# ConwayBeyond/Funscript-Flow

Measured on AMD Instinct MI355X. Metric: 1080p frame-pairs/sec, higher is better.
Workload: dtype f32

## Files before the change

### funscript_flow_amd/csrc/ffl_api.hip

```cpp
#include "../../include/ffl.h"
#include "ffl_kernels.h"

#include <math.h>
#include <stdarg.h>
#include <stdio.h>
#include <string.h>

#include <algorithm>
#include <condition_variable>
#include <mutex>
#include <string>
#include <thread>
#include <vector>

#define FFL_EV_RING 16
#define FFL_RAW_RING 4

template <class H, class Arg, hipError_t (*Free)(Arg)>
struct Owned {
    H h = H();
    Owned() = default;
    explicit Owned(H take) : h(take) {}
    Owned(Owned &&o) noexcept : h(o.release()) {}
    Owned &operator=(Owned &&o) noexcept { std::swap(h, o.h); return *this; }
// ... 671 lines not shown
            HIPCHK(c, hipMemcpyAsync(rb.d, rb.h, fbytes, hipMemcpyHostToDevice, c->s_copy));
        }
        {
            ProfScope ps(c, FFL_K_FRONTEND, c->s_copy);
            if (rp) ffl_launch_frontend_remap(desc(rb.d), c->d_gray + (size_t)fs * c->N, fp, *rp, c->s_copy);
            else ffl_launch_frontend(desc(rb.d), c->d_gray + (size_t)fs * c->N, fp, c->s_copy);
        }
        HIPCHK(c, hipEventRecord(rb.ev, c->s_copy));
        rb.busy = true;
    }
    return publish_frames(c, first, n);
}

extern "C" {

int ffl_device_count(void) {
    int n = 0;
    if (hipGetDeviceCount(&n) != hipSuccess) return 0;
    return n;
}

const char *ffl_last_error(const ffl_ctx *ctx) {
    if (!ctx) return g_create_error.c_str();
    static thread_local std::string copy;
    CtxLock lk(ctx->mu);
    copy = ctx->err;
    return copy.c_str();
}

const char *ffl_kernel_name(int k) {
    static const char *names[FFL_K_COUNT] = {"k_gray",  "k_pyr_level", "k_polyexp", "k_frontend",
                                             "k_update_matrices", "k_blur_solve", "k_pass1", "k_radial"};
    return (k >= 0 && k < FFL_K_COUNT) ? names[k] : "?";
}

void ffl_destroy(ffl_ctx *c) {
    if (!c) return;
    hipSetDevice(c->device);
    for (auto &L : c->lanes)
        if (L.st) hipStreamSynchronize(L.st);
    if (c->s_post) hipStreamSynchronize(c->s_post);
    if (c->s_copy) hipStreamSynchronize(c->s_copy);
    prof_collect(c);
    c->pool.shutdown();
    delete c;
}

static int create_resources(ffl_ctx *c) {
    const int width = c->w, height = c->h, n_frame_slots = c->n_fslots, n_flow_slots = c->n_slots;
    const int num_lanes = c->opt.lanes;
    const Geometry &geo = c->geo;
    const Layout &lay = c->lay;
    HIPCHK(nullptr, hipSetDevice(c->device));
    int prio_least = 0, prio_greatest = 0;
    HIPCHK(nullptr, hipDeviceGetStreamPriorityRange(&prio_least, &prio_greatest));
    HIPCHK(nullptr, hipStreamCreateWithPriority(c->s_copy.put(), hipStreamNonBlocking, prio_greatest));
    HIPCHK(nullptr, hipStreamCreateWithPriority(c->s_post.put(), hipStreamNonBlocking, prio_greatest));
    HIPCHK_ALLOC(nullptr, hipMalloc, c->d_gray, lay.gray + 16);
    HIPCHK_ALLOC(nullptr, hipMalloc, c->d_bgr, lay.bgr);
    HIPCHK_ALLOC(nullptr, hipHostMalloc, c->h_stage_gray, lay.gray, hipHostMallocDefault);
    HIPCHK_ALLOC(nullptr, hipHostMalloc, c->h_stage_bgr, lay.bgr, hipHostMallocDefault);
    c->p1_blocks = ffl_pass1_blocks(width, height);
    c->lanes.resize(num_lanes);
    for (auto &L : c->lanes) {
        HIPCHK(nullptr, hipStreamCreateWithFlags(L.st.put(), hipStreamNonBlocking));
        HIPCHK(nullptr, L.ring.create(FFL_EV_RING));
        HIPCHK_ALLOC(nullptr, hipMalloc, L.d_I, lay.I);
        HIPCHK_ALLOC(nullptr, hipMalloc, L.d_T, lay.T);
        HIPCHK_ALLOC(nullptr, hipMalloc, L.d_R, lay.R);
        for (auto &M : L.d_M) HIPCHK_ALLOC(nullptr, hipMalloc, M, lay.M);
        HIPCHK_ALLOC(nullptr, hipMalloc, L.d_flowA, lay.flow);
        HIPCHK_ALLOC(nullptr, hipMalloc, L.d_flowB, lay.flow);
        HIPCHK_ALLOC(nullptr, hipMalloc, L.d_pkey, lay.p1);
        HIPCHK_ALLOC(nullptr, hipMalloc, L.d_psum, lay.p1);
        HIPCHK_ALLOC(nullptr, hipMalloc, L.d_tab, 1);
        HIPCHK_ALLOC(nullptr, hipHostMalloc, L.h_tab, lay.tab, hipHostMallocDefault);
        for (int k = geo.levels; k >= 0; k--, L.n_jobs++) {
            const LevelGeom &g = geo.lv[k];
            const size_t plane = (size_t)g.lw * g.lh;
            PyrJob &P = L.pyr[L.n_jobs];
            P.w = width; P.h = height; P.lw = g.lw; P.lh = g.lh;
            P.sx = (double)width / g.lw; P.sy = (double)height / g.lh;
            P.gk = g.gk;
            P.tmp = L.d_T + lay.t_off[k]; P.tmp_stride = ffl_pyr_tmp_floats(width, height, g.lw);
            P.I = L.d_I + lay.i_off[k]; P.I_stride = plane;
            PolyJob &Q = L.poly[L.n_jobs];
            Q.I = P.I; Q.I_stride = plane;
            Q.R = L.d_R + lay.r_off[k]; Q.R_stride = 5 * plane; Q.plane = plane;
            Q.w = g.lw; Q.h = g.lh;
        }
    }
    HIPCHK_ALLOC(nullptr, hipMalloc, c->d_flow, lay.slots);
    HIPCHK_ALLOC(nullptr, hipHostMalloc, c->h_res, lay.res, hipHostMallocMapped);
    HIPCHK(nullptr, hipHostGetDevicePointer((void **)&c->d_res, c->h_res, 0));
    HIPCHK_ALLOC(nullptr, hipMalloc, c->d_rpsum, (size_t)c->p1_blocks * FFL_MAXB);
    {
        std::vector<double> wy(2 * (size_t)height);
        for (int y = 0; y < height; y++) {
            wy[y] = (double)(height - y) / (double)height;
            wy[height + y] = (double)y / (double)height;
        }
        HIPCHK_ALLOC(nullptr, hipMalloc, c->d_wytab, wy.size());
        HIPCHK(nullptr, hipMemcpy(c->d_wytab, wy.data(), sizeof(double) * wy.size(), hipMemcpyHostToDevice));
    }
    HIPCHK_ALLOC(nullptr, hipMalloc, c->d_wtab, FFL_MAXB);
    HIPCHK_ALLOC(nullptr, hipHostMalloc, c->h_wtab, FFL_MAXB, hipHostMallocDefault);
// ... 2175 lines not shown
        ProfScope ps(c, FFL_K_PASS1, st);
        ffl_launch_pass1(c->d_ptab, 1, c->w, c->h, pov_mode, c->d_pskey, c->d_rpsum, st);
    }
    EvRef done;
    if (int rc = publish_post(c, 1, &slot, &done)) return rc;
    HIPCHK(c, hipGetLastError());
    return FFL_OK;
}

int ffl_submit_pair(ffl_ctx *c, int slot, const uint8_t *prev, const uint8_t *next, int width, int height, int channels,
                    ptrdiff_t stride_bytes, int pov_mode) {
    if (!c) return FFL_ERR_INVALID;
    if (!flow_slot_ok(c, slot) || 2 * slot + 1 >= c->n_fslots) {
        CtxLock lk(c->mu);
        return set_err(c, FFL_ERR_INVALID, "ffl_submit_pair: slot %d needs frame slots %d,%d and a flow slot", slot, 2 * slot, 2 * slot + 1);
    }
    int rc = ffl_upload_frame(c, 2 * slot, prev, width, height, channels, stride_bytes);
    if (rc) return rc;
    rc = ffl_upload_frame(c, 2 * slot + 1, next, width, height, channels, stride_bytes);
    if (rc) return rc;
    int f0 = 2 * slot, f1 = 2 * slot + 1;
    return ffl_flow_pairs(c, 1, &f0, &f1, &slot, pov_mode);
}

int ffl_sync(ffl_ctx *c) {
    if (!c) return FFL_ERR_INVALID;
    std::unique_lock<std::mutex> ul(c->up_mu);
    std::unique_lock<std::mutex> pl(c->post_mu);
    CtxLock lk(c->mu);
    std::vector<hipEvent_t> evs;
    evs.push_back(ev_latest(c->up_ring).get());
    for (auto &rb : c->raw)
        if (rb.busy) evs.push_back(rb.ev);
    for (auto &L : c->lanes) evs.push_back(ev_latest(L.ring).get());
    evs.push_back(ev_latest(c->post_ring).get());
    pl.unlock();
    ul.unlock();
    return wait_unlocked(c, lk, evs.data(), (int)evs.size());
}

static constexpr struct { const char *name; int value; } kFixedKnobs[] = {
    {"blur_tile_h", 16}, {"run_ahead", 0}, {"merge_expand", 1}};
static const int *fixed_knob(const char *name) {
    for (const auto &k : kFixedKnobs)
        if (!strcmp(name, k.name)) return &k.value;
    return nullptr;
}
static const FflOptionRow *option_row(const char *name) {
    for (const FflOptionRow &r : kFflOptionRows)
        if (!strcmp(name, r.name)) return &r;
    return nullptr;
}

static int set_option_impl(FflOptions &o, const char *name, int value, bool live) {
    if (const int *fixed = fixed_knob(name)) return value == *fixed ? FFL_OK : FFL_ERR_INVALID;
    const FflOptionRow *r = option_row(name);
    if (!r || value < r->lo || value > r->hi) return FFL_ERR_INVALID;
    if (live && r->member == &FflOptions::lanes) return value == o.lanes ? FFL_OK : FFL_ERR_STATE;
    o.*r->member = r->flag ? value != 0 : value;
    return FFL_OK;
}

static int get_option_impl(const FflOptions &o, const char *name, int *value) {
    const int *fixed = fixed_knob(name);
    const FflOptionRow *r = option_row(name);
    if (!fixed && !r) return FFL_ERR_INVALID;
    *value = fixed ? *fixed : o.*r->member;
    return FFL_OK;
}

int ffl_set_option(const char *name, int value) {
    if (!name) return FFL_ERR_INVALID;
    std::lock_guard<std::mutex> g(g_opt_mu);
    return set_option_impl(g_opts, name, value, false);
}

int ffl_ctx_set_option(ffl_ctx *c, const char *name, int value) {
    if (!c || !name) return FFL_ERR_INVALID;
    CtxLock lk(c->mu);
    const int rc = set_option_impl(c->opt, name, value, true);
    if (rc == FFL_OK) c->opt_epoch++;
    else if (rc == FFL_ERR_STATE) set_err(c, rc, "ffl_ctx_set_option: \"lanes\" is fixed once the context exists (%d)", c->opt.lanes);
    else set_err(c, rc, "ffl_ctx_set_option: unknown option or value out of range: %s = %d", name, value);
    return rc;
}

int ffl_ctx_get_option(ffl_ctx *c, const char *name, int *value) {
    if (!name || !value) return FFL_ERR_INVALID;
    if (!c) {
        std::lock_guard<std::mutex> g(g_opt_mu);
        return get_option_impl(g_opts, name, value);
    }
    CtxLock lk(c->mu);
    return get_option_impl(c->opt, name, value);
}

int ffl_graph_stats(ffl_ctx *c, int *captured, int *replayed, int *capture_failures) {
    if (!c) return FFL_ERR_INVALID;
    CtxLock lk(c->mu);
    if (captured) *captured = c->graph_captured;
    if (replayed) *replayed = c->graph_replayed;
    if (capture_failures) *capture_failures = c->graph_failed;
    return FFL_OK;
}

int ffl_profile_enable(ffl_ctx *c, unsigned class_mask) {
    if (!c) return FFL_ERR_INVALID;
    int rc = ffl_sync(c);
    if (rc) return rc;
    CtxLock lk(c->mu);
    prof_collect(c);
    c->prof_mask = class_mask;
    return FFL_OK;
}

int ffl_profile_read(ffl_ctx *c, int k, int *launches, double *total_ms) {
// ... 14 lines not shown
```

### funscript_flow_amd/csrc/ffl_kernels.h

```cpp
#pragma once
#include <hip/hip_runtime.h>
#include <limits.h>
#include <stdint.h>

#define FFL_MAXB 256
#define FFL_MAXU (2 * FFL_MAXB)
#define FFL_MAX_LEVELS 4
#define FFL_POLY_N 5
#define FFL_WIN 15
#define FFL_WIN_R 7

struct PolyConsts {
    float g[FFL_POLY_N + 1], xg[FFL_POLY_N + 1], xxg[FFL_POLY_N + 1];
    double gd[FFL_POLY_N + 1], xxgd[FFL_POLY_N + 1];
    double ig11, ig03, ig33, ig55;
};

struct GaussKernel {
    float k[32];
    int ksize;
};

struct UTab {
    int fslot[FFL_MAXU];
};

struct PairTab {
    int u0[FFL_MAXB], u1[FFL_MAXB];
    float *flow[FFL_MAX_LEVELS][FFL_MAXB];
    struct Pass1Result *res[FFL_MAXB];
};

struct BatchTab {
    UTab ut;
    PairTab pt;
};

struct Pass1Result {
    int x, y;
    float div_val;
    int weighted;
    double mag_sum;
};
__host__ __device__ inline double ffl_record_mean(const Pass1Result &r, double npx) {
    return r.weighted ? r.mag_sum : r.mag_sum / npx;
}

enum { FFL_FRONT_GENERIC = 0, FFL_FRONT_AREA2 = 1, FFL_FRONT_IDENTITY = 2 };
enum { FFL_SRC_GRAY = 0, FFL_SRC_BGR = 1, FFL_SRC_YUV = 2, FFL_SRC_YUV16 = 3, FFL_SRC_ANY = -1 };
struct FrameDesc {
    const uint8_t *p0, *p1, *p2;
    long long pitch0, pitch1, pitch2;
    long long ps, cs;
    int c_step;
    int wx, wy;
    int fslot;
// ... 12 lines not shown
#define FFL_REMAP_NONE (-2147483647 - 1)
struct RemapParams {
    const int2 *map;
    int ss, lg;
};
struct ExportTab {
    int slot[FFL_MAXB];
};

enum { FFL_IMP_F32 = 0, FFL_IMP_F16 = 1, FFL_IMP_BF16 = 2 };
enum { FFL_IMP_ANY = 0,
       FFL_IMP_NHWC = 1,
       FFL_IMP_NCHW = 2 };
struct ImportArgs {
    const char *base;
    long long item, pitch, ps, cs;
    float *flow;
    Pass1Result *res;
};

struct WeightArgs {
    const char *base;
    long long item, pitch;
};

#define FFL_MAX_JOBS 4
enum { FFL_PYR_NONE = -1, FFL_PYR_F1 = 0, FFL_PYR_F2, FFL_PYR_H4, FFL_PYR_H9, FFL_PYR_V4, FFL_PYR_V9, FFL_PYR_H1 };
struct PyrJob {
    int kind, w, h, lw, lh;
    unsigned gx, gy, first, count;
    double sx, sy;
    float *tmp, *I;
    size_t tmp_stride, I_stride;
    GaussKernel gk;
};
struct PyrJobs {
    PyrJob j[FFL_MAX_JOBS];
    int n;
};
struct PolyJob {
    const float *I;
    float *R;
    size_t I_stride, R_stride, plane;
    int w, h;
    unsigned gx, gy, first, count;
    int from_gray;
    float gk0, gk1;
};
struct PolyJobs {
    PolyJob j[FFL_MAX_JOBS];
    int n;
};

struct FflOptions {
    int lanes = 2;
    int fuse_first = 10000;
    int use_graph = 1;
    int copy_threads = 4;
    int blur_rows = 0;
    int blur_min_wgs = 3500;
    int tile_order = 0;
    int pyr_coarse = 1;
    int fuse_l0_blur = 1;
    int fb_general = 0;
};
struct FflOptionRow {
    const char *name;
    int FflOptions::*member;
    int lo, hi;
    bool flag;
};
inline constexpr FflOptionRow kFflOptionRows[] = {
    {"lanes", &FflOptions::lanes, 1, 4, false},
    {"fuse_first", &FflOptions::fuse_first, 0, INT_MAX, false},
    {"graph", &FflOptions::use_graph, INT_MIN, INT_MAX, true},
    {"copy_threads", &FflOptions::copy_threads, 1, 16, false},
    {"blur_rows", &FflOptions::blur_rows, 0, 64, false},
    {"blur_min_wgs", &FflOptions::blur_min_wgs, 1, INT_MAX, false},
    {"tile_order", &FflOptions::tile_order, 0, 1, false},
    {"pyr_coarse", &FflOptions::pyr_coarse, INT_MIN, INT_MAX, true},
    {"fuse_l0_blur", &FflOptions::fuse_l0_blur, INT_MIN, INT_MAX, true},
    {"fb_general", &FflOptions::fb_general, 0, 1, false},
};

bool ffl_launch_pyr_multi(const uint8_t *gray_base, size_t gray_stride, const UTab *ut, int nU, const PyrJob *levels, int n,
                          const FflOptions &opt, hipStream_t st);
bool ffl_polyexp_from_gray_ok(const PyrJob &l0);
void ffl_launch_polyexp_multi(const PolyJob *levels, int n, int nU, PolyConsts pc, const uint8_t *gray_base, size_t gray_stride,
                              const UTab *ut, const PyrJob *l0, hipStream_t st);
void ffl_launch_frontend(const FrameDesc &d, uint8_t *gray, const FrontParams &p, hipStream_t st);
void ffl_launch_frontend_dev(const FrameDesc *tab, int n, uint8_t *gray_base, size_t N, const FrontParams &p, hipStream_t st);
void ffl_launch_frontend_remap(const FrameDesc &d, uint8_t *gray, const FrontParams &p, const RemapParams &r, hipStream_t st);
void ffl_launch_frontend_remap_dev(const FrameDesc *tab, int n, uint8_t *gray_base, size_t N, const FrontParams &p,
                                   const RemapParams &r, hipStream_t st);
void ffl_launch_export_flows(const float *flow, const ExportTab &tab, int n, size_t N, char *dst, long long item_stride,
                             int layout, hipStream_t st);
void ffl_launch_import_pass1(const ImportArgs &a, const ExportTab &tab, int n, int dtype, int mode, int w, int h, int pov_mode,
                             PairTab *pt, unsigned long long *pkey, double *psum, hipStream_t st);
void ffl_launch_gray(const uint8_t *bgr, uint8_t *gray, int n_pixels, hipStream_t st);
size_t ffl_pyr_tmp_floats(int w, int h, int lw);
bool ffl_pyr_level_ok(int w, int h, int lw, int lh, int ksize);
void ffl_launch_pyr_level(const uint8_t *gray_base, size_t gray_stride, const UTab *ut, int nU, const PyrJob &level,
                          hipStream_t st);
void ffl_launch_update_matrices(const float *R, size_t R_stride, size_t plane, const PairTab *pt, int level, int nB, float *M,
                                size_t M_stride, int lw, int lh, int pw, int ph, int zero_flow, int store_flow,
                                const FflOptions &opt, hipStream_t st);
void ffl_launch_blur_solve(const float *Min, float *Mout, size_t M_stride, const float *R, size_t R_stride,
                           size_t plane, const PairTab *pt, int level, int nB, int lw, int lh, int update, int store_flow,
                           const FflOptions &opt, hipStream_t st);


void ffl_launch_blur_solve_first(float *Mout, size_t M_stride, const float *R, size_t R_stride, size_t plane,
                                 const PairTab *pt, int level, int nB, int lw, int lh, int pw, int ph, const FflOptions &opt,
                                 hipStream_t st);

#define DIS_MAX_PATCHES 4096
#define DIS_MAX_SCALES 12
struct DisKParams {
    int w, h, finest, coarsest, stride, gd_iters, vr_iters, mean_norm, spatial_prop, stripes;
    float alpha, gamma, delta;
    size_t pair_floats;
    size_t pyr_floats;
    size_t pyr_off[DIS_MAX_SCALES];
    float *dbg;
    int dbg_scale, dbg_stage;
};
void ffl_launch_dis(const UTab *ut, const PairTab *pt, int nB, const uint8_t *gray, size_t gray_stride, float *scratch,
                    const DisKParams &p, hipStream_t st);

int ffl_pass1_blocks(int w, int h);
void ffl_launch_pass1(const PairTab *pt, int nB, int w, int h, int pov_mode, unsigned long long *pkey, double *psum,
                      hipStream_t st);

#define FFL_WINDOW_MAX_RADIUS 32
struct WindowSeq {
    int slot[FFL_MAXB + 2 * FFL_WINDOW_MAX_RADIUS];
};
struct WindowItem {
    const float *flow;
    double cx, cy;
    int cut, pad;
};
struct Pass2Record {
    double dot, cx, cy;
    float mean_mag, div_val;
    int x, y, cut, pad;
};
struct AxesRecord {
    Pass2Record base;
    double tangential, shift_x, shift_y, reserved;
};
#define FFL_NAXES 4
int ffl_radial_blocks(int w, int h);
struct RadialForm {
    int nc;
    const WeightArgs *maps;
// ... 95 lines not shown
        } else {
            const double za1 = Sux - l10 * Su, za2 = (Suy - l20 * Su) - l21 * za1;
            const double zb1 = Svx - l10 * Sv, zb2 = (Svy - l20 * Sv) - l21 * zb1;
            r.a2 = za2 / d2;
            r.a1 = za1 / d1 - l21 * r.a2;
            r.a0 = (ta - l10 * r.a1) - l20 * r.a2;
            r.b2 = zb2 / d2;
            r.b1 = zb1 / d1 - l21 * r.b2;
            r.b0 = (tb - l10 * r.b1) - l20 * r.b2;
        }
    }
    *out = r;
}

void ffl_launch_motion_fit(const float *flow, const ExportTab &tab, int n, int w, int h, const WeightArgs *maps,
                           const MotionPrior &prior, float tau, int model, double *psum, MotionRecord *models, double *sums,
                           hipStream_t st);
void ffl_launch_motion_subtract(float *flow, Pass1Result *res, const ExportTab &src, const ExportTab &dst, int n, int w, int h,
                                const char *models, long long stride, PairTab *pt, hipStream_t st);

__device__ __forceinline__ int ffl_clampi(int v, int lo, int hi) { return v < lo ? lo : (v > hi ? hi : v); }

__device__ __forceinline__ int ffl_reflect101(int p, int n) {
    if (n == 1) return 0;
    while (p < 0 || p >= n) p = p < 0 ? -p : 2 * (n - 1) - p;
    return p;
}

__device__ __forceinline__ void ffl_resize_coord(int d, int src, double scale, int &i0, int &i1, float &f) {
    float fx = (float)((d + 0.5) * scale - 0.5);
    int sx = (int)floorf(fx);
    fx -= sx;
    if (sx < 0) { sx = 0; fx = 0.f; }
    if (sx >= src - 1) { sx = src - 1; fx = 0.f; }
    i0 = sx;
    i1 = sx + 1 < src ? sx + 1 : src - 1;
    f = fx;
}

static inline unsigned ffl_xcd_blocks(unsigned count) { return ((count + 7) / 8) * 8; }
__device__ __forceinline__ bool ffl_xcd_tile(unsigned l, unsigned count, unsigned &t) {
    const unsigned chunk = (count + 7) >> 3;
    t = (l & 7u) * chunk + (l >> 3);
    return (l >> 3) < chunk && t < count;
}

#ifndef FFL_PANEL_W
#define FFL_PANEL_W 4
#endif
static inline unsigned ffl_tile_grid(int tiles_x, int tiles_y, int nB) {
    const int T = tiles_x * tiles_y;
    return (unsigned)(((T + 7) / 8) * 8 * nB);
}
__device__ __forceinline__ bool ffl_tile_coord(int tiles_x, int tiles_y, int nB, int order, int &b, int &tile_x,
                                               int &tile_y) {
    const int T = tiles_x * tiles_y, chunk = (T + 7) >> 3;
    int t;
    if (order == 0) {
        b = blockIdx.x / (chunk * 8);
        const int l = blockIdx.x - b * (chunk * 8);
        t = (l & 7) * chunk + (l >> 3);
    } else {
        const int pos = blockIdx.x >> 3, tt = pos / nB;
        b = pos - tt * nB;
        t = (blockIdx.x & 7) * chunk + tt;
    }
    if (t >= T) return false;
    const int per_panel = FFL_PANEL_W * tiles_y;
    const int panel = t / per_panel, within = t - panel * per_panel;
    const int pw = min(FFL_PANEL_W, tiles_x - panel * FFL_PANEL_W);
    tile_y = within / pw;
    tile_x = panel * FFL_PANEL_W + (within - tile_y * pw);
    return true;
}

#define FFL_GLOBAL __attribute__((address_space(1)))
typedef float ffl_v2f __attribute__((ext_vector_type(2), aligned(4)));
typedef float ffl_v4f __attribute__((ext_vector_type(4), aligned(4)));
__device__ __forceinline__ float2 ffl_gload2(const void *base, size_t byte_off) {
    const ffl_v2f v = *(const FFL_GLOBAL ffl_v2f *)((const char *)base + byte_off);
    return make_float2(v.x, v.y);
}
__device__ __forceinline__ float4 ffl_gload4(const void *base, size_t byte_off) {
    const ffl_v4f v = *(const FFL_GLOBAL ffl_v4f *)((const char *)base + byte_off);
    return make_float4(v.x, v.y, v.z, v.w);
}

struct __attribute__((packed, aligned(4))) ffl_f2u { float x, y; };
struct __attribute__((packed, aligned(4))) ffl_f4u { float x, y, z, w; };

template <typename T>
__device__ __forceinline__ const T *ffl_at(const float *base, unsigned idx) {
    return reinterpret_cast<const T *>(reinterpret_cast<const char *>(base) + idx * 4u);
}
template <typename T>
__device__ __forceinline__ T *ffl_at(float *base, unsigned idx) {
    return reinterpret_cast<T *>(reinterpret_cast<char *>(base) + idx * 4u);
}

__device__ __forceinline__ ffl_f2u ffl_ld_corner(const float *plane_base, unsigned idx) {
    ffl_f2u v;
    v.x = *ffl_at<float>(plane_base, idx);
    v.y = *ffl_at<float>(plane_base, idx + 1u);
    return v;
}

struct UmLoc {
    int x1, y1;
    float a00, a01, a10, a11;
    bool inside;
};
__device__ __forceinline__ UmLoc ffl_um_locate(int w, int h, int x, int y, float dx, float dy) {
    UmLoc L;
    float fx = x + dx, fy = y + dy;
    L.x1 = (int)floorf(fx);
    L.y1 = (int)floorf(fy);
    fx -= L.x1;
    fy -= L.y1;
    L.inside = (unsigned)L.x1 < (unsigned)(w - 1) && (unsigned)L.y1 < (unsigned)(h - 1);
    L.a00 = (1.f - fx) * (1.f - fy);
    L.a01 = fx * (1.f - fy);
    L.a10 = (1.f - fx) * fy;
    L.a11 = fx * fy;
    return L;
}

// ... 62 lines not shown
```

### funscript_flow_amd/csrc/kernels_farneback.hip

```cpp
#include "ffl_kernels.h"

__global__ __launch_bounds__(256) void k_gray(const uint8_t *__restrict__ bgr, uint8_t *__restrict__ gray, int n) {
    int i4 = (blockIdx.x * 256 + threadIdx.x) * 4;
    if (i4 + 3 < n) {
        const uint32_t *p = reinterpret_cast<const uint32_t *>(bgr + (size_t)i4 * 3);
        uint32_t a = p[0], b = p[1], c = p[2];
        uint32_t px[12] = {a & 255, (a >> 8) & 255, (a >> 16) & 255, a >> 24, b & 255, (b >> 8) & 255,
                           (b >> 16) & 255, b >> 24, c & 255, (c >> 8) & 255, (c >> 16) & 255, c >> 24};
        uint32_t o = 0;
#pragma unroll
        for (int j = 0; j < 4; j++) {
            uint32_t g = (px[j * 3] * 3735u + px[j * 3 + 1] * 19235u + px[j * 3 + 2] * 9798u + 16384u) >> 15;
            o |= g << (8 * j);
        }
        *reinterpret_cast<uint32_t *>(gray + i4) = o;
    } else {
        for (int i = i4; i < n; i++) {
            uint32_t b = bgr[(size_t)i * 3], g = bgr[(size_t)i * 3 + 1], r = bgr[(size_t)i * 3 + 2];
            gray[i] = (uint8_t)((b * 3735u + g * 19235u + r * 9798u + 16384u) >> 15);
        }
    }
}

void ffl_launch_gray(const uint8_t *bgr, uint8_t *gray, int n_pixels, hipStream_t st) {
// ... 797 lines not shown
    if (!ffl_tile_coord((w + 63) / 64, (h + 15) / 16, nB, order, b, tile_x, tile_y)) return;
    const int lx = threadIdx.x & 63, x0 = tile_x * 64, x = min(x0 + lx, w - 1);
    const bool xin = x0 + lx < w;
    const float *R0 = R + (size_t)pt->u0[b] * R_stride, *R1 = R + (size_t)pt->u1[b] * R_stride;
    float *flow = pt->flow[level][b];
    const float *pf = pt->flow[min(level + 1, FFL_MAX_LEVELS - 1)][b];
    constexpr int NR = 4;
    const int ybase = tile_y * 16 + (threadIdx.x >> 6);
    float2 f[NR];
    if (MODE == 1) {
        const bool half_scale = usx == 0.5 && usy == 0.5;
        int xa0, xa1;
        float a1;
        if (half_scale) ffl_resize_coord_half(x, pw, xa0, xa1, a1);
        else ffl_resize_coord(x, pw, usx, xa0, xa1, a1);
        const int xq = min(xa0, pw - 2);
        float4 c0[NR], c1[NR];
        float b1[NR];
#pragma unroll
        for (int k = 0; k < NR; k++) {
            int ya0, ya1;
            const int y = min(ybase + 4 * k, h - 1);
            if (half_scale) ffl_resize_coord_half(y, ph, ya0, ya1, b1[k]);
            else ffl_resize_coord(y, ph, usy, ya0, ya1, b1[k]);
            c0[k] = ffl_gload4(pf, 8u * ((unsigned)ya0 * (unsigned)pw + xq));
            c1[k] = ffl_gload4(pf, 8u * ((unsigned)ya1 * (unsigned)pw + xq));
        }
#pragma unroll
        for (int k = 0; k < NR; k++) f[k] = ffl_upsample2(c0[k], c1[k], xa0 == xq, xa1 == xq, a1, b1[k]);
    } else if (MODE == 0) {
#pragma unroll
        for (int k = 0; k < NR; k++) {
            const unsigned o = (unsigned)min(ybase + 4 * k, h - 1) * (unsigned)w + (unsigned)x;
            const FFL_GLOBAL float *q = (const FFL_GLOBAL float *)flow + 2u * o;
            f[k] = make_float2(q[0], q[1]);
        }
    } else {
#pragma unroll
        for (int k = 0; k < NR; k++) f[k] = make_float2(0.f, 0.f);
    }
    ffl_um_rows<NR>(R0, R1, M + (size_t)b * M_stride, plane, w, h, x, xin, ybase, [&](int k) { return f[k]; },
                    [&](unsigned o, float2 d) {
                        if (MODE == 1 && store_flow) {
                            flow[2u * o] = d.x;
                            flow[2u * o + 1u] = d.y;
                        }
                    });
}

void ffl_launch_update_matrices(const float *R, size_t R_stride, size_t plane, const PairTab *pt, int level, int nB,
                                float *M,
                                size_t M_stride, int lw, int lh, int pw, int ph, int zero_flow, int store_flow,
                                const FflOptions &opt, hipStream_t st) {
    dim3 grid(ffl_tile_grid((lw + 63) / 64, (lh + 15) / 16, nB));
    const auto k = pw > 0 ? k_update_matrices<1> : (zero_flow ? k_update_matrices<2> : k_update_matrices<0>);
    hipLaunchKernelGGL(k, grid, dim3(256), 0, st, R, R_stride, plane, pt, level, M, M_stride, lw, lh, pw, ph,
                       pw > 0 ? (double)pw / lw : 1.0, pw > 0 ? (double)ph / lh : 1.0, pw > 0 ? store_flow : 0, nB,
                       opt.tile_order);
}

#ifndef FFL_K5_WAVES
#define FFL_K5_WAVES 4
#endif
#ifndef FFL_K5_WAVES_FIRST
#define FFL_K5_WAVES_FIRST 3
#endif
#ifndef FFL_K5_GROUP_FIRST
#define FFL_K5_GROUP_FIRST 3
#endif
#ifndef FFL_K5_GROUP
#define FFL_K5_GROUP 3
#endif

__device__ __forceinline__ void ffl_box_block16(const float (&v)[30], double (&out)[16]) {
    double s[15];
    s[14] = (double)v[14];
#pragma unroll
    for (int j = 13; j >= 0; j--) s[j] = (double)v[j] + s[j + 1];
    double p = (double)v[15];
    out[0] = s[0];
#pragma unroll
    for (int t = 1; t < 15; t++) {
        out[t] = s[t] + p;
        p = p + (double)v[15 + t];
    }
    out[15] = p;
}

template <int Q>
__device__ __forceinline__ void ffl_box_quarter(const double (&d)[18], double (&out)[4]) {
    constexpr int NA = 15 - 4 * Q;
    double S[4] = {0.0, 0.0, 0.0, 0.0};
    double s = d[NA - 1];
    if (NA - 1 < 4) S[NA - 1] = s;
#pragma unroll
    for (int j = NA - 2; j >= 0; j--) {
        s = d[j] + s;
        if (j < 4) S[j] = s;
    }
    double p = d[NA];
#pragma unroll
    for (int m = 0; m <= 4 * Q + 2; m++) {
        if (m > 0) p = p + d[NA + m];
        const int i = m + 1 - 4 * Q;
        if (i >= 0 && i < 4) {
            if (4 * Q + i == 15) out[i] = p;
            else out[i] = S[i] + p;
        }
    }
    if (Q == 0) out[0] = S[0];
}

#ifdef FFL_STAMP
#define FFL_NSTAMP 16
__device__ unsigned long long g_stamp[64][FFL_NSTAMP];
extern "C" int ffl_debug_read_stamps(unsigned long long *out) {
    return (int)hipMemcpyFromSymbol(out, HIP_SYMBOL(g_stamp), sizeof(unsigned long long) * 64 * FFL_NSTAMP);
}
#define FFL_T(i)                                                              \
    if (FFL_STAMP_ON && tid == 0) {                                           \
        const unsigned long long t_ = __builtin_readcyclecounter();          \
        sStamp[i] += t_ - sStamp[FFL_NSTAMP];                                 \
        sStamp[FFL_NSTAMP] = t_;                                              \
    }
#else
#define FFL_T(i)
#endif


template <bool UPDATE, int FIRST>
__global__ __launch_bounds__(256, FIRST ? FFL_K5_WAVES_FIRST : FFL_K5_WAVES) void k_blur_solve(
    const float *__restrict__ Min, float *__restrict__ Mout, size_t M_stride, const float *__restrict__ R, size_t R_stride,
    size_t plane, const PairTab *__restrict__ pt, int level, int w, int h, int nrb, int pw, int ph, double usx, double usy,
    int store_flow, int nB,
    int order) {
    constexpr int TW = 64, TH = 16, LW = TW + 2 * FFL_WIN_R, LH = TH + 2 * FFL_WIN_R;
    constexpr int PX = 4;
    constexpr int NCARRY = LH - TH;
    constexpr int LW2 = 44;
    constexpr int GC = FIRST ? FFL_K5_GROUP_FIRST : FFL_K5_GROUP, NG = (5 + GC - 1) / GC;
    __shared__ double2 sS2[GC][TH][LW2];
    const int tid = threadIdx.x;
#ifdef FFL_STAMP
    __shared__ unsigned long long sStamp[FFL_NSTAMP + 1];
    const bool FFL_STAMP_ON = FIRST == 1 && w >= 1024;
    if (FFL_STAMP_ON && tid == 0) {
        for (int i = 0; i < FFL_NSTAMP; i++) sStamp[i] = 0;
        sStamp[FFL_NSTAMP] = __builtin_readcyclecounter();
    }
#endif
    int b, tile_x, strip_y;
    const int tiles_y = (h + TH - 1) / TH;
    if (!ffl_tile_coord((w + TW - 1) / TW, (tiles_y + nrb - 1) / nrb, nB, order, b, tile_x, strip_y)) return;
    const int x0 = tile_x * TW;
    const float *Mb = Min + (size_t)b * M_stride;

    const int q = __builtin_amdgcn_readfirstlane(tid >> 6);
    const int ty = (tid & 63) >> 2, kk = tid & 3;
    const int lx0 = 16 * kk + 4 * q;
    double *sS = reinterpret_cast<double *>(&sS2[0][0][0]);
    const int vcc = tid / LW, vtx = tid - vcc * LW;
    const int vgx = min(max(x0 + vtx - FFL_WIN_R, 0), w - 1);
    const unsigned pitch = (unsigned)w * 4u;
    float carry[NG][NCARRY];
    const double scale = 1.0 / (FFL_WIN * FFL_WIN);
    float2 *flow = reinterpret_cast<float2 *>(pt->flow[level][b]);
    const float *R0 = R + (size_t)pt->u0[b] * R_stride, *R1 = R + (size_t)pt->u1[b] * R_stride;
    float *Mo = Mout + (size_t)b * M_stride;
    constexpr int FP = TW + 2;
    float4 *sF4 = reinterpret_cast<float4 *>(&sS2[0][0][0]);
    constexpr int UP = 80;
    __shared__ float sM34[FIRST ? 5 - GC : 1][FIRST ? TH : 1][FIRST ? UP : 1];
    float *sM012 = reinterpret_cast<float *>(&sS2[0][0][0]);
    static_assert(GC * TH * UP * 4 <= (int)sizeof(sS2), "the first group's staged rows must fit the column sums");
    const float2 *prevf = reinterpret_cast<const float2 *>(pt->flow[min(level + 1, FFL_MAX_LEVELS - 1)][b]);
    struct UStageA {
        float a1, b1;
        float4 c0, c1;
        bool first0, first1;
        int r, tx, gx, gy;
    };
    const bool half_scale = usx == 0.5 && usy == 0.5;
    auto phase_u = [&](int y0, int jbase, int nrows) {
        const int N = LW * nrows;
        auto coords = [&](int i, int &r, int &tx, int &gx, int &gy) {
            r = i / LW;
            tx = i - r * LW;
            gy = min(max(y0 - FFL_WIN_R + jbase + r, 0), h - 1);
            gx = min(max(x0 + tx - FFL_WIN_R, 0), w - 1);
        };
        auto issue = [&](int i) {
            UStageA A;
            coords(i, A.r, A.tx, A.gx, A.gy);
            const int gx = A.gx, gy = A.gy;
            if (FIRST == 1) {
                int xa0, xa1, ya0, ya1;
                if (half_scale) {
                    ffl_resize_coord_half(gx, pw, xa0, xa1, A.a1);
                    ffl_resize_coord_half(gy, ph, ya0, ya1, A.b1);
                } else {
                    ffl_resize_coord(gx, pw, usx, xa0, xa1, A.a1);
                    ffl_resize_coord(gy, ph, usy, ya0, ya1, A.b1);
                }
                const float *pf = reinterpret_cast<const float *>(prevf);
                const unsigned r0o = (unsigned)ya0 * (unsigned)pw, r1o = (unsigned)ya1 * (unsigned)pw;
                const int xq = min(xa0, pw - 2);
                A.c0 = ffl_gload4(pf, 8u * (r0o + xq));
                A.c1 = ffl_gload4(pf, 8u * (r1o + xq));
                A.first0 = xa0 == xq;
                A.first1 = xa1 == xq;
            }
            return A;
        };
        int i = tid;
        if (i >= N) return;
        UStageA A = issue(i);
#pragma unroll 1
        for (;;) {
            const int r = A.r, tx = A.tx, gx = A.gx, gy = A.gy;
            const int inext = i + 256;
            const bool more = inext < N;
            float2 f = make_float2(0.f, 0.f);
            if (FIRST == 1) f = ffl_upsample2(A.c0, A.c1, A.first0, A.first1, A.a1, A.b1);
            float r0[5];
            {
                const unsigned o = (unsigned)gy * (unsigned)w + (unsigned)gx;
#pragma unroll
                for (int c = 0; c < 5; c++) r0[c] = *ffl_at<float>(R0 + c * plane, o);
            }
            const UmLoc L = ffl_um_locate(w, h, gx, gy, f.x, f.y);
            const unsigned o1 = L.inside ? (unsigned)L.y1 * (unsigned)w + (unsigned)L.x1 : 0u;
            ffl_f2u t[5], u[5];
#pragma unroll
            for (int c = 0; c < 5; c++) {
                t[c] = ffl_ld_corner(R1 + c * plane, o1);
                u[c] = ffl_ld_corner(R1 + c * plane, o1 + (unsigned)w);
            }
            const UStageA Anext = issue(more ? inext : i);
            float b[5];
#pragma unroll
            for (int c = 0; c < 5; c++) b[c] = L.a00 * t[c].x + L.a01 * t[c].y + L.a10 * u[c].x + L.a11 * u[c].y;
            float m[5];
            ffl_um_finish(r0, b, L.inside, w, h, gx, gy, f.x, f.y, m);
#pragma unroll
            for (int c = 0; c < GC; c++) sM012[(c * TH + r) * UP + tx] = m[c];
#pragma unroll
            for (int c = GC; c < 5; c++) sM34[c - GC][r][tx] = m[c];
            if (!more) break;
            A = Anext;
            i = inext;
        }
    };

#pragma unroll 1
    for (int rb = 0; rb < nrb; rb++) {
        const int y0 = (strip_y * nrb + rb) * TH;
        if (y0 >= h) break;
        double acc[5][PX];
        if (FIRST) {
            if (rb == 0) {
                phase_u(y0, 0, NCARRY);
                __syncthreads();
#pragma unroll
                for (int g = 0; g < NG; g++) {
                    const int c0 = g * GC, nc = min(GC, 5 - c0);
                    if (tid < nc * LW) {
#pragma unroll
                        for (int j = 0; j < NCARRY; j++)
                            carry[g][j] = g == 0 ? sM012[(vcc * TH + j) * UP + vtx] : sM34[c0 - GC + vcc][j][vtx];
                    }
                }
                __syncthreads();
            }
            FFL_T(0)
            phase_u(y0, NCARRY, TH);
            FFL_T(1)
            __syncthreads();
            FFL_T(2)
        }
#pragma unroll
        for (int g = 0; g < NG; g++) {
            const int c0 = g * GC, nc = min(GC, 5 - c0);
            if (g) __syncthreads();
            FFL_T(3)
            const bool vlane = tid < nc * LW;
            float v[LH];
            if (vlane) {
                const char *Mbb = reinterpret_cast<const char *>(Mb);
                const unsigned lane_byte = ((unsigned)((c0 + vcc) * plane) + (unsigned)vgx) * 4u;
                if (FIRST) {
#pragma unroll
                    for (int j = 0; j < NCARRY; j++) v[j] = carry[g][j];
#pragma unroll
                    for (int j = 0; j < TH; j++)
                        v[NCARRY + j] = g == 0 ? sM012[(vcc * TH + j) * UP + vtx] : sM34[c0 - GC + vcc][j][vtx];
                } else {
                    if (rb == 0) {
#pragma unroll
                        for (int j = 0; j < NCARRY; j++) {
                            const unsigned gy = (unsigned)min(max(y0 + j - FFL_WIN_R, 0), h - 1);
                            v[j] = *reinterpret_cast<const float *>(Mbb + (gy * pitch + lane_byte));
                        }
                    } else {
#pragma unroll
                        for (int j = 0; j < NCARRY; j++) v[j] = carry[g][j];
                    }
#pragma unroll
                    for (int j = NCARRY; j < LH; j++) {
                        const unsigned gy = (unsigned)min(max(y0 + j - FFL_WIN_R, 0), h - 1);
// ... 45 lines not shown
            float2 f[PX];
#pragma unroll
            for (int p = 0; p < PX; p++) {
                double g11 = acc[0][p] * scale, g12 = acc[1][p] * scale, g22 = acc[2][p] * scale,
                       h1 = acc[3][p] * scale, h2 = acc[4][p] * scale;
                double idet = 1.0 / (g11 * g22 - g12 * g12 + 1e-3);
                f[p].x = (float)((g11 * h2 - g12 * h1) * idet);
                f[p].y = (float)((g22 * h1 - g12 * h2) * idet);
            }
            sF4[(ty * FP + lx0) / 2] = make_float4(f[0].x, f[0].y, f[1].x, f[1].y);
            sF4[(ty * FP + lx0) / 2 + 1] = make_float4(f[2].x, f[2].y, f[3].x, f[3].y);
        }
        FFL_T(8)
        __syncthreads();
        FFL_T(9)
        if (UPDATE) {
            const int lx = tid & 63, x = min(x0 + lx, w - 1);
            const float2 *sF2 = reinterpret_cast<const float2 *>(sF4);
            ffl_um_rows<TH / 4>(R0, R1, Mo, plane, w, h, x, x0 + lx < w, y0 + (tid >> 6),
                                [&](int k) { return sF2[((tid >> 6) + 4 * k) * FP + lx]; },
                                [&](unsigned o, float2 d) {
                                    if (store_flow) *reinterpret_cast<float2 *>(ffl_at<float>(reinterpret_cast<float *>(flow), 2u * o)) = d;
                                });
        } else {
            const int lx = 2 * (tid & 31), x = x0 + lx;
            if (x < w) {
                const bool second = x + 1 < w;
#pragma unroll
                for (int k = 0; k < TH / 8; k++) {
                    const int ly = (tid >> 5) + 8 * k;
                    if (y0 + ly >= h) continue;
                    const float4 ff = sF4[(ly * FP + lx) >> 1];
                    const size_t o = (size_t)(y0 + ly) * w + x;
                    if (second) {
                        ffl_f4u t;
                        t.x = ff.x; t.y = ff.y; t.z = ff.z; t.w = ff.w;
                        *reinterpret_cast<ffl_f4u *>(flow + o) = t;
                    } else {
                        flow[o] = make_float2(ff.x, ff.y);
                    }
                }
            }
        }
        FFL_T(10)
        __syncthreads();
        FFL_T(11)
    }
#ifdef FFL_STAMP
    if (FFL_STAMP_ON && tid == 0)
        for (int i = 0; i < FFL_NSTAMP; i++) g_stamp[blockIdx.x & 63][i] = sStamp[i];
#endif
}

static int ffl_blur_rows_per_wg(int tiles_x, int tiles_y, int nB, int min_wgs) {
    if (nB > 32 && tiles_x * tiles_y >= 256) nB = 32;
    for (int s = 1; s <= tiles_y; s++) {
        const int nrb = (tiles_y + s - 1) / s;
        if (nrb > 64) continue;
        if ((long)tiles_x * ((tiles_y + nrb - 1) / nrb) * nB >= min_wgs || nrb == 1) return nrb;
    }
    return 1;
}

template <typename K>
static void ffl_launch_k5(K k, const float *Min, float *Mout, size_t M_stride, const float *R, size_t R_stride, size_t plane,
                          const PairTab *pt, int level, int nB, int lw, int lh, int pw, int ph, int store_flow,
                          const FflOptions &opt, hipStream_t st) {
    const int tiles_x = (lw + 63) / 64, tiles_y = (lh + 15) / 16;
    const int nrb = opt.blur_rows > 0 ? opt.blur_rows : ffl_blur_rows_per_wg(tiles_x, tiles_y, nB, opt.blur_min_wgs);
    dim3 grid(ffl_tile_grid(tiles_x, (tiles_y + nrb - 1) / nrb, nB));
    hipLaunchKernelGGL(k, grid, dim3(256), 0, st, Min, Mout, M_stride, R, R_stride, plane, pt, level, lw, lh, nrb, pw, ph,
                       pw > 0 ? (double)pw / lw : 1.0, pw > 0 ? (double)ph / lh : 1.0, store_flow, nB, opt.tile_order);
}

void ffl_launch_blur_solve(const float *Min, float *Mout, size_t M_stride, const float *R, size_t R_stride,
                           size_t plane, const PairTab *pt, int level, int nB, int lw, int lh, int update, int store_flow,
                           const FflOptions &opt, hipStream_t st) {
    ffl_launch_k5(update ? k_blur_solve<true, 0> : k_blur_solve<false, 0>, Min, Mout, M_stride, R, R_stride, plane, pt, level,
                  nB, lw, lh, 0, 0, update ? store_flow : 1, opt, st);
}

void ffl_launch_blur_solve_first(float *Mout, size_t M_stride, const float *R, size_t R_stride, size_t plane,
                                 const PairTab *pt, int level, int nB, int lw, int lh, int pw, int ph, const FflOptions &opt,
                                 hipStream_t st) {
    ffl_launch_k5(pw > 0 ? k_blur_solve<true, 1> : k_blur_solve<true, 2>, (const float *)nullptr, Mout, M_stride, R, R_stride,
                  plane, pt, level, nB, lw, lh, pw, ph, 0, opt, st);
}
```

Baseline: 6492.

## Plan blur-solve row strips with an occupancy-aware cost model

Replaces the fixed threshold heuristic for rows-per-workgroup in the blur/solve kernel with a planner. The planner queries device occupancy per kernel and models per-chunk load imbalance and drain cost, allowing two strip heights so that tail strips are balanced. It also adds a force option for manual plans. The goal is better work distribution across CUs and less tail idling. The cost is extra host-side planning per launch and a slightly more complex block-to-tile mapping in the kernel.

```diff
diff --git a/funscript_flow_amd/csrc/ffl_api.hip b/funscript_flow_amd/csrc/ffl_api.hip
--- a/funscript_flow_amd/csrc/ffl_api.hip
+++ b/funscript_flow_amd/csrc/ffl_api.hip
@@ -747,6 +747,10 @@
     const Geometry &geo = c->geo;
     const Layout &lay = c->lay;
     HIPCHK(nullptr, hipSetDevice(c->device));
+    HIPCHK(nullptr, ffl_query_strip_slots(c->device, c->opt.strip_slots));
+    for (int i = 0; i < FFL_SLOT_COUNT; i++)
+        if (c->opt.strip_slots[i] < 1)
+            return set_err(nullptr, FFL_ERR_HIP, "ffl_create: the device holds no workgroup of tile kernel %s", kFflSlotNames[i] + 6);
     int prio_least = 0, prio_greatest = 0;
     HIPCHK(nullptr, hipDeviceGetStreamPriorityRange(&prio_least, &prio_greatest));
     HIPCHK(nullptr, hipStreamCreateWithPriority(c->s_copy.put(), hipStreamNonBlocking, prio_greatest));
@@ -3028,16 +3032,39 @@
     return nullptr;
 }
 
+static int set_strip_force(FflOptions &o, int value) {
+    if (value < 0) return FFL_ERR_INVALID;
+    const int level = (value >> 25) & 7, kind = (value >> 23) & 3, layout = value & ((1 << FFL_STRIP_FORCE_BITS) - 1);
+    if (value >> 28 || level > FFL_MAX_LEVELS || (layout & 127) > FFL_STRIP_MAX_TILES || ((layout >> 15) & 127) > FFL_STRIP_MAX_TILES)
+        return FFL_ERR_INVALID;
+    for (int l = 0; l < FFL_MAX_LEVELS; l++)
+        for (int k = 0; k < 3; k++)
+            if (value == 0 || ((level == 0 || level == l + 1) && (kind == 3 || kind == k))) o.strip_force[l][k] = layout;
+    o.strip_force_last = value;
+    return FFL_OK;
+}
+
 static int set_option_impl(FflOptions &o, const char *name, int value, bool live) {
     if (const int *fixed = fixed_knob(name)) return value == *fixed ? FFL_OK : FFL_ERR_INVALID;
+    if (!strcmp(name, "strip_force")) return set_strip_force(o, value);
     const FflOptionRow *r = option_row(name);
     if (!r || value < r->lo || value > r->hi) return FFL_ERR_INVALID;
     if (live && r->member == &FflOptions::lanes) return value == o.lanes ? FFL_OK : FFL_ERR_STATE;
     o.*r->member = r->flag ? value != 0 : value;
+    if (r->member == &FflOptions::blur_min_wgs) o.strip_plan = 0;
     return FFL_OK;
 }
 
 static int get_option_impl(const FflOptions &o, const char *name, int *value) {
+    if (!strcmp(name, "strip_force")) {
+        *value = o.strip_force_last;
+        return FFL_OK;
+    }
+    for (int i = 0; i < FFL_SLOT_COUNT; i++)
+        if (!strcmp(name, kFflSlotNames[i])) {
+            *value = o.strip_slots[i];
+            return FFL_OK;
+        }
     const int *fixed = fixed_knob(name);
     const FflOptionRow *r = option_row(name);
     if (!fixed && !r) return FFL_ERR_INVALID;
diff --git a/funscript_flow_amd/csrc/ffl_kernels.h b/funscript_flow_amd/csrc/ffl_kernels.h
--- a/funscript_flow_amd/csrc/ffl_kernels.h
+++ b/funscript_flow_amd/csrc/ffl_kernels.h
@@ -2,6 +2,7 @@
 #include <hip/hip_runtime.h>
 #include <limits.h>
 #include <stdint.h>
+#include "ffl_strip_plan.h"
 
 #define FFL_MAXB 256
 #define FFL_MAXU (2 * FFL_MAXB)
@@ -120,6 +121,18 @@
     int n;
 };
 
+enum { FFL_SLOT_K5_FIRST_UP = 0,
+       FFL_SLOT_K5_FIRST_ZERO,
+       FFL_SLOT_K5_UPDATE,
+       FFL_SLOT_K5_LAST,
+       FFL_SLOT_UM_READ,
+       FFL_SLOT_UM_UP,
+       FFL_SLOT_UM_ZERO,
+       FFL_SLOT_COUNT };
+inline constexpr const char *kFflSlotNames[FFL_SLOT_COUNT] = {
+    "slots_blur_first_up", "slots_blur_first_zero", "slots_blur_update", "slots_blur_last",
+    "slots_um_read", "slots_um_up", "slots_um_zero"};
+
 struct FflOptions {
     int lanes = 2;
     int fuse_first = 10000;
@@ -127,11 +140,16 @@
     int copy_threads = 4;
     int blur_rows = 0;
     int blur_min_wgs = 3500;
+    int strip_plan = 1;
     int tile_order = 0;
     int pyr_coarse = 1;
     int fuse_l0_blur = 1;
     int fb_general = 0;
-};
+    int strip_force[FFL_MAX_LEVELS][3] = {};
+    int strip_force_last = 0;
+    int strip_slots[FFL_SLOT_COUNT] = {};
+};
+#define FFL_STRIP_FORCE_BITS 23
 struct FflOptionRow {
     const char *name;
     int FflOptions::*member;
@@ -145,6 +163,7 @@
     {"copy_threads", &FflOptions::copy_threads, 1, 16, false},
     {"blur_rows", &FflOptions::blur_rows, 0, 64, false},
     {"blur_min_wgs", &FflOptions::blur_min_wgs, 1, INT_MAX, false},
+    {"strip_plan", &FflOptions::strip_plan, 0, 1, false},
     {"tile_order", &FflOptions::tile_order, 0, 1, false},
     {"pyr_coarse", &FflOptions::pyr_coarse, INT_MIN, INT_MAX, true},
     {"fuse_l0_blur", &FflOptions::fuse_l0_blur, INT_MIN, INT_MAX, true},
@@ -170,6 +189,7 @@
 bool ffl_pyr_level_ok(int w, int h, int lw, int lh, int ksize);
 void ffl_launch_pyr_level(const uint8_t *gray_base, size_t gray_stride, const UTab *ut, int nU, const PyrJob &level,
                           hipStream_t st);
+hipError_t ffl_query_strip_slots(int device, int *slots);
 void ffl_launch_update_matrices(const float *R, size_t R_stride, size_t plane, const PairTab *pt, int level, int nB, float *M,
                                 size_t M_stride, int lw, int lh, int pw, int ph, int zero_flow, int store_flow,
                                 const FflOptions &opt, hipStream_t st);
@@ -371,18 +391,18 @@
     const int T = tiles_x * tiles_y;
     return (unsigned)(((T + 7) / 8) * 8 * nB);
 }
-__device__ __forceinline__ bool ffl_tile_coord(int tiles_x, int tiles_y, int nB, int order, int &b, int &tile_x,
-                                               int &tile_y) {
+__device__ __forceinline__ bool ffl_tile_coord_at(int bid, int tiles_x, int tiles_y, int nB, int order, int &b, int &tile_x,
+                                                  int &tile_y) {
     const int T = tiles_x * tiles_y, chunk = (T + 7) >> 3;
     int t;
     if (order == 0) {
-        b = blockIdx.x / (chunk * 8);
-        const int l = blockIdx.x - b * (chunk * 8);
+        b = bid / (chunk * 8);
+        const int l = bid - b * (chunk * 8);
         t = (l & 7) * chunk + (l >> 3);
     } else {
-        const int pos = blockIdx.x >> 3, tt = pos / nB;
+        const int pos = bid >> 3, tt = pos / nB;
         b = pos - tt * nB;
-        t = (blockIdx.x & 7) * chunk + tt;
+        t = (bid & 7) * chunk + tt;
     }
     if (t >= T) return false;
     const int per_panel = FFL_PANEL_W * tiles_y;
@@ -391,6 +411,10 @@
     tile_y = within / pw;
     tile_x = panel * FFL_PANEL_W + (within - tile_y * pw);
     return true;
+}
+__device__ __forceinline__ bool ffl_tile_coord(int tiles_x, int tiles_y, int nB, int order, int &b, int &tile_x,
+                                               int &tile_y) {
+    return ffl_tile_coord_at((int)blockIdx.x, tiles_x, tiles_y, nB, order, b, tile_x, tile_y);
 }
 
 #define FFL_GLOBAL __attribute__((address_space(1)))
diff --git a/funscript_flow_amd/csrc/ffl_strip_plan.h b/funscript_flow_amd/csrc/ffl_strip_plan.h
--- /dev/null
+++ b/funscript_flow_amd/csrc/ffl_strip_plan.h
@@ -0,0 +1,121 @@
+#pragma once
+
+#define FFL_STRIP_MAX_TILES 64
+
+enum {
+    FFL_STRIP_FIRST = 0,
+    FFL_STRIP_UPDATE = 1,
+    FFL_STRIP_LAST = 2,
+    FFL_STRIP_UM = 3,
+    FFL_STRIP_KINDS = 4
+};
+
+struct FflStripPlan {
+    int n1, s1, n2, s2;
+    unsigned first2;
+    unsigned grid;
+};
+
+static inline unsigned ffl_strip_blocks(int tiles_x, int strips, int nB) {
+    const int T = tiles_x * strips;
+    return (unsigned)(((T + 7) / 8) * 8 * nB);
+}
+
+static inline FflStripPlan ffl_strip_finish(int tiles_x, int nB, int n1, int s1, int n2, int s2, int tail) {
+    FflStripPlan p;
+    p.n1 = n1, p.s1 = s1, p.n2 = n2, p.s2 = s2;
+    if (tail && s2 > 0) {
+        p.first2 = ffl_strip_blocks(tiles_x, s1, nB);
+        p.grid = p.first2 + ffl_strip_blocks(tiles_x, s2, nB);
+    } else {
+        p.first2 = 0;
+        p.grid = ffl_strip_blocks(tiles_x, s1 + s2, nB);
+    }
+    return p;
+}
+
+static inline FflStripPlan ffl_strip_plan_rows(int tiles_x, int tiles_y, int nB, int nrb) {
+    if (nrb < 1) nrb = 1;
+    if (nrb > FFL_STRIP_MAX_TILES) nrb = FFL_STRIP_MAX_TILES;
+    return ffl_strip_finish(tiles_x, nB, nrb, (tiles_y + nrb - 1) / nrb, nrb, 0, 0);
+}
+
+static inline int ffl_strip_rows_threshold(int tiles_x, int tiles_y, int nB, int min_wgs) {
+    if (nB > 32 && tiles_x * tiles_y >= 256) nB = 32;
+    for (int s = 1; s <= tiles_y; s++) {
+        const int nrb = (tiles_y + s - 1) / s;
+        if (nrb > FFL_STRIP_MAX_TILES) continue;
+        if ((long)tiles_x * ((tiles_y + nrb - 1) / nrb) * nB >= min_wgs || nrb == 1) return nrb;
+    }
+    return 1;
+}
+
+static inline FflStripPlan ffl_strip_plan_forced(int tiles_x, int tiles_y, int nB, int n1, int s1, int n2, int tail) {
+    const auto clamp = [](int n) { return n < 1 ? 1 : (n > FFL_STRIP_MAX_TILES ? FFL_STRIP_MAX_TILES : n); };
+    n1 = clamp(n1), n2 = clamp(n2);
+    const int all1 = (tiles_y + n1 - 1) / n1;
+    if (s1 < 1) s1 = 1;
+    if (s1 > all1) s1 = all1;
+    const int rest = tiles_y - s1 * n1;
+    const int s2 = rest > 0 ? (rest + n2 - 1) / n2 : 0;
+    return ffl_strip_finish(tiles_x, nB, n1, s1, n2, s2, tail);
+}
+
+#ifndef FFL_PANEL_W
+#define FFL_PANEL_W 4
+#endif
+#define FFL_STRIP_MIN_ROUNDS 3.0
+#define FFL_STRIP_MIN_DEPTH 10.0
+struct FflStripModel {
+    double start, drain;
+};
+static inline FflStripModel ffl_strip_model(int kind) {
+    switch (kind) {
+        case FFL_STRIP_FIRST: return {1.0, 1.0};
+        case FFL_STRIP_UPDATE: return {0.8, 0.5};
+        default: return {0.3, 0.1};
+    }
+}
+
+static inline double ffl_strip_work_before(int t, int tiles_x, int S, int s1, double c1, double c2) {
+    const auto prefix = [&](int k) { return k <= s1 ? k * c1 : s1 * c1 + (k - s1) * c2; };
+    const int per_panel = FFL_PANEL_W * S, panel = t / per_panel, within = t - panel * per_panel;
+    const int pw = tiles_x - panel * FFL_PANEL_W < FFL_PANEL_W ? tiles_x - panel * FFL_PANEL_W : FFL_PANEL_W;
+    const double whole = (double)panel * FFL_PANEL_W * prefix(S);
+    if (pw <= 0) return whole;
+    const int sy = within / pw, col = within - sy * pw;
+    return whole + pw * prefix(sy) + col * (sy < s1 ? c1 : c2);
+}
+
+static inline double ffl_strip_cost(const FflStripModel &m, int tiles_x, int nB, int slots, int n1, int s1, int n2, int s2) {
+    const int S = s1 + s2, T = tiles_x * S, chunk = (T + 7) / 8;
+    const double c1 = n1 + m.start, c2 = n2 + m.start;
+    double most = 0;
+    for (int x = 0; x < 8; x++) {
+        const int lo = x * chunk < T ? x * chunk : T, hi = (x + 1) * chunk < T ? (x + 1) * chunk : T;
+        const double w = ffl_strip_work_before(hi, tiles_x, S, s1, c1, c2) - ffl_strip_work_before(lo, tiles_x, S, s1, c1, c2);
+        if (w > most) most = w;
+    }
+    const double L = c1 > c2 || s2 == 0 ? c1 : c2;
+    double t = nB * most / (slots / 8.0);
+    if (t < L) t = L;
+    return t + m.drain * L;
+}
+
+static inline FflStripPlan ffl_strip_plan(int tiles_x, int tiles_y, int nB, int slots, int kind) {
+    if (kind == FFL_STRIP_UM) return ffl_strip_finish(tiles_x, nB, 1, tiles_y, 1, 0, 0);
+    if (slots < 8) slots = 8;
+    const FflStripModel m = ffl_strip_model(kind);
+    int bn1 = 1, bs1 = tiles_y, bn2 = 1, bs2 = 0;
+    double best = -1;
+    if ((double)tiles_x * tiles_y * nB < FFL_STRIP_MIN_DEPTH * slots) return ffl_strip_finish(tiles_x, nB, 1, tiles_y, 1, 0, 0);
+    for (int S = 1; S <= tiles_y; S++) {
+        const int n1 = (tiles_y + S - 1) / S;
+        if (n1 > FFL_STRIP_MAX_TILES) continue;
+        if ((double)tiles_x * S * nB < FFL_STRIP_MIN_ROUNDS * slots) continue;
+        const int s2 = S * n1 - tiles_y, s1 = S - s2, n2 = s2 ? n1 - 1 : n1;
+        const double t = ffl_strip_cost(m, tiles_x, nB, slots, n1, s1, n2, s2);
+        if (best < 0 || t < best) best = t, bn1 = n1, bs1 = s1, bn2 = n2, bs2 = s2;
+    }
+    return ffl_strip_finish(tiles_x, nB, bn1, bs1, bn2, bs2, 0);
+}
diff --git a/funscript_flow_amd/csrc/kernels_farneback.hip b/funscript_flow_amd/csrc/kernels_farneback.hip
--- a/funscript_flow_amd/csrc/kernels_farneback.hip
+++ b/funscript_flow_amd/csrc/kernels_farneback.hip
@@ -873,7 +873,8 @@
                                 float *M,
                                 size_t M_stride, int lw, int lh, int pw, int ph, int zero_flow, int store_flow,
                                 const FflOptions &opt, hipStream_t st) {
-    dim3 grid(ffl_tile_grid((lw + 63) / 64, (lh + 15) / 16, nB));
+    const int slot = pw > 0 ? FFL_SLOT_UM_UP : (zero_flow ? FFL_SLOT_UM_ZERO : FFL_SLOT_UM_READ);
+    dim3 grid(ffl_strip_plan((lw + 63) / 64, (lh + 15) / 16, nB, opt.strip_slots[slot], FFL_STRIP_UM).grid);
     const auto k = pw > 0 ? k_update_matrices<1> : (zero_flow ? k_update_matrices<2> : k_update_matrices<0>);
     hipLaunchKernelGGL(k, grid, dim3(256), 0, st, R, R_stride, plane, pt, level, M, M_stride, lw, lh, pw, ph,
                        pw > 0 ? (double)pw / lw : 1.0, pw > 0 ? (double)ph / lh : 1.0, pw > 0 ? store_flow : 0, nB,
@@ -952,9 +953,8 @@
 template <bool UPDATE, int FIRST>
 __global__ __launch_bounds__(256, FIRST ? FFL_K5_WAVES_FIRST : FFL_K5_WAVES) void k_blur_solve(
     const float *__restrict__ Min, float *__restrict__ Mout, size_t M_stride, const float *__restrict__ R, size_t R_stride,
-    size_t plane, const PairTab *__restrict__ pt, int level, int w, int h, int nrb, int pw, int ph, double usx, double usy,
-    int store_flow, int nB,
-    int order) {
+    size_t plane, const PairTab *__restrict__ pt, int level, int w, int h, FflStripPlan sp, int pw, int ph, double usx,
+    double usy, int store_flow, int nB, int order) {
     constexpr int TW = 64, TH = 16, LW = TW + 2 * FFL_WIN_R, LH = TH + 2 * FFL_WIN_R;
     constexpr int PX = 4;
     constexpr int NCARRY = LH - TH;
@@ -971,8 +971,15 @@
     }
 #endif
     int b, tile_x, strip_y;
-    const int tiles_y = (h + TH - 1) / TH;
-    if (!ffl_tile_coord((w + TW - 1) / TW, (tiles_y + nrb - 1) / nrb, nB, order, b, tile_x, strip_y)) return;
+    {
+        const bool second = sp.first2 != 0 && blockIdx.x >= sp.first2;
+        const int bid = (int)blockIdx.x - (second ? (int)sp.first2 : 0);
+        const int strips = sp.first2 != 0 ? (second ? sp.s2 : sp.s1) : sp.s1 + sp.s2;
+        if (!ffl_tile_coord_at(bid, (w + TW - 1) / TW, strips, nB, order, b, tile_x, strip_y)) return;
+        if (second) strip_y += sp.s1;
+    }
+    const int nrb = strip_y < sp.s1 ? sp.n1 : sp.n2;
+    const int tile_y0 = strip_y < sp.s1 ? strip_y * sp.n1 : sp.s1 * sp.n1 + (strip_y - sp.s1) * sp.n2;
     const int x0 = tile_x * TW;
     const float *Mb = Min + (size_t)b * M_stride;
 
@@ -1075,7 +1082,7 @@
 
 #pragma unroll 1
     for (int rb = 0; rb < nrb; rb++) {
-        const int y0 = (strip_y * nrb + rb) * TH;
+        const int y0 = (tile_y0 + rb) * TH;
         if (y0 >= h) break;
         double acc[5][PX];
         if (FIRST) {
@@ -1227,37 +1234,57 @@
 #endif
 }
 
-static int ffl_blur_rows_per_wg(int tiles_x, int tiles_y, int nB, int min_wgs) {
-    if (nB > 32 && tiles_x * tiles_y >= 256) nB = 32;
-    for (int s = 1; s <= tiles_y; s++) {
-        const int nrb = (tiles_y + s - 1) / s;
-        if (nrb > 64) continue;
-        if ((long)tiles_x * ((tiles_y + nrb - 1) / nrb) * nB >= min_wgs || nrb == 1) return nrb;
-    }
-    return 1;
+static FflStripPlan ffl_k5_plan(int tiles_x, int tiles_y, int nB, int level, int kind, int slot, const FflOptions &opt) {
+    const int f = level >= 0 && level < FFL_MAX_LEVELS ? opt.strip_force[level][kind] : 0;
+    if (f & 127) return ffl_strip_plan_forced(tiles_x, tiles_y, nB, f & 127, (f >> 7) & 255, (f >> 15) & 127, (f >> 22) & 1);
+    if (opt.blur_rows > 0) return ffl_strip_plan_rows(tiles_x, tiles_y, nB, opt.blur_rows);
+    if (!opt.strip_plan)
+        return ffl_strip_plan_rows(tiles_x, tiles_y, nB, ffl_strip_rows_threshold(tiles_x, tiles_y, nB, opt.blur_min_wgs));
+    return ffl_strip_plan(tiles_x, tiles_y, nB, opt.strip_slots[slot], kind);
 }
 
 template <typename K>
-static void ffl_launch_k5(K k, const float *Min, float *Mout, size_t M_stride, const float *R, size_t R_stride, size_t plane,
-                          const PairTab *pt, int level, int nB, int lw, int lh, int pw, int ph, int store_flow,
+static void ffl_launch_k5(K k, int kind, int slot, const float *Min, float *Mout, size_t M_stride, const float *R, size_t R_stride,
+                          size_t plane, const PairTab *pt, int level, int nB, int lw, int lh, int pw, int ph, int store_flow,
                           const FflOptions &opt, hipStream_t st) {
-    const int tiles_x = (lw + 63) / 64, tiles_y = (lh + 15) / 16;
-    const int nrb = opt.blur_rows > 0 ? opt.blur_rows : ffl_blur_rows_per_wg(tiles_x, tiles_y, nB, opt.blur_min_wgs);
-    dim3 grid(ffl_tile_grid(tiles_x, (tiles_y + nrb - 1) / nrb, nB));
-    hipLaunchKernelGGL(k, grid, dim3(256), 0, st, Min, Mout, M_stride, R, R_stride, plane, pt, level, lw, lh, nrb, pw, ph,
+    const FflStripPlan sp = ffl_k5_plan((lw + 63) / 64, (lh + 15) / 16, nB, level, kind, slot, opt);
+    hipLaunchKernelGGL(k, dim3(sp.grid), dim3(256), 0, st, Min, Mout, M_stride, R, R_stride, plane, pt, level, lw, lh, sp, pw, ph,
                        pw > 0 ? (double)pw / lw : 1.0, pw > 0 ? (double)ph / lh : 1.0, store_flow, nB, opt.tile_order);
 }
 
 void ffl_launch_blur_solve(const float *Min, float *Mout, size_t M_stride, const float *R, size_t R_stride,
                            size_t plane, const PairTab *pt, int level, int nB, int lw, int lh, int update, int store_flow,
                            const FflOptions &opt, hipStream_t st) {
-    ffl_launch_k5(update ? k_blur_solve<true, 0> : k_blur_solve<false, 0>, Min, Mout, M_stride, R, R_stride, plane, pt, level,
-                  nB, lw, lh, 0, 0, update ? store_flow : 1, opt, st);
+    if (update)
+        ffl_launch_k5(k_blur_solve<true, 0>, FFL_STRIP_UPDATE, FFL_SLOT_K5_UPDATE, Min, Mout, M_stride, R, R_stride, plane, pt,
+                      level, nB, lw, lh, 0, 0, store_flow, opt, st);
+    else
+        ffl_launch_k5(k_blur_solve<false, 0>, FFL_STRIP_LAST, FFL_SLOT_K5_LAST, Min, Mout, M_stride, R, R_stride, plane, pt,
+                      level, nB, lw, lh, 0, 0, 1, opt, st);
 }
 
 void ffl_launch_blur_solve_first(float *Mout, size_t M_stride, const float *R, size_t R_stride, size_t plane,
                                  const PairTab *pt, int level, int nB, int lw, int lh, int pw, int ph, const FflOptions &opt,
                                  hipStream_t st) {
-    ffl_launch_k5(pw > 0 ? k_blur_solve<true, 1> : k_blur_solve<true, 2>, (const float *)nullptr, Mout, M_stride, R, R_stride,
+    ffl_launch_k5(pw > 0 ? k_blur_solve<true, 1> : k_blur_solve<true, 2>, FFL_STRIP_FIRST,
+                  pw > 0 ? FFL_SLOT_K5_FIRST_UP : FFL_SLOT_K5_FIRST_ZERO, (const float *)nullptr, Mout, M_stride, R, R_stride,
                   plane, pt, level, nB, lw, lh, pw, ph, 0, opt, st);
 }
+
+hipError_t ffl_query_strip_slots(int device, int *slots) {
+    int cus = 0;
+    hipError_t e = hipDeviceGetAttribute(&cus, hipDeviceAttributeMultiprocessorCount, device);
+    const auto ask = [&](auto kernel, int slot) {
+        int per_cu = 0;
+        if (e == hipSuccess) e = hipOccupancyMaxActiveBlocksPerMultiprocessor(&per_cu, kernel, 256, 0);
+        slots[slot] = per_cu * cus;
+    };
+    ask(k_blur_solve<true, 1>, FFL_SLOT_K5_FIRST_UP);
+    ask(k_blur_solve<true, 2>, FFL_SLOT_K5_FIRST_ZERO);
+    ask(k_blur_solve<true, 0>, FFL_SLOT_K5_UPDATE);
+    ask(k_blur_solve<false, 0>, FFL_SLOT_K5_LAST);
+    ask(k_update_matrices<0>, FFL_SLOT_UM_READ);
+    ask(k_update_matrices<1>, FFL_SLOT_UM_UP);
+    ask(k_update_matrices<2>, FFL_SLOT_UM_ZERO);
+    return e;
+}
```

Result: no change. 6468 (-0.4%).
